# linusmossberg/monte-carlo-ray-tracer

Hardware: NVIDIA H100
Metric: Mray/s (primary+shadow+bounce) (higher is better)
Workload: dtype f64

## Files before the change

include/mcrt_abi.h:

```cpp
#ifndef MCRT_ABI_H
#define MCRT_ABI_H

#include <stddef.h>
#include <stdint.h>

#ifdef __cplusplus
extern "C" {
#endif

#define MCRT_ABI_VERSION 1

typedef enum mcrt_status {
    MCRT_OK = 0,
    MCRT_ERR_INVALID = -1,
    MCRT_ERR_CUDA = -2,
    MCRT_ERR_NO_SCENE = -3,
    MCRT_ERR_UNSUPPORTED = -4,
    MCRT_ERR_NO_PHOTONS = -5
} mcrt_status;

enum { MCRT_PRIM_TRIANGLE = 0, MCRT_PRIM_SPHERE = 1, MCRT_PRIM_QUADRIC = 2 };

enum { MCRT_INTEGRATOR_PATH = 0, MCRT_INTEGRATOR_PHOTON = 1 };

// ... 47 lines not shown
    const uint32_t* light_prim;
    const double* light_cdf;
    double scene_ior;
} mcrt_scene_desc;

typedef struct mcrt_camera {
    double eye[3], forward[3], left[3], up[3];
    double focal_length, sensor_width, aperture_radius, focus_distance;
    uint32_t width, height;
    uint32_t thin_lens;
    uint32_t _pad;
} mcrt_camera;

typedef struct mcrt_ray {
    double origin[3];
    double direction[3];
} mcrt_ray;

typedef struct mcrt_hit {
    double t, u, v;
    uint32_t prim;
    uint32_t interpolate;
} mcrt_hit;

typedef struct mcrt_photon_map_desc {
    uint32_t n_octants;
    const double* octant_bounds;
    const uint64_t* octant_start;
    const uint64_t* octant_count;
    const uint32_t* octant_next_sibling;
    const uint8_t* octant_leaf;
    uint64_t n_photons;
    const float* photons;
} mcrt_photon_map_desc;

typedef struct mcrt_stats {
    uint64_t paths;
    uint64_t extension_rays;
    uint64_t shadow_rays;
    uint64_t box_tests;
    uint64_t prim_tests;
    uint64_t knn_queries;
    uint64_t wavefront_iterations;
    uint64_t kernel_launches;
    uint64_t ior_stack_overflows;
    uint32_t max_depth;
    uint32_t _pad;
    double gpu_ms_total;
    double gpu_ms_generate, gpu_ms_extend, gpu_ms_shade, gpu_ms_shadow, gpu_ms_knn;
    uint64_t extend_launches, shadow_launches;
    uint64_t shadow_box_tests, shadow_prim_tests;
    uint64_t extend_work_sum, extend_work_warpmax;
    uint64_t replayed_rays;
} mcrt_stats;

typedef struct mcrt_ctx mcrt_ctx;

int mcrt_abi_version(void);

int mcrt_init(int device, mcrt_ctx** out_ctx);
void mcrt_destroy(mcrt_ctx* ctx);
const char* mcrt_last_error(const mcrt_ctx* ctx);

int mcrt_scene_upload(mcrt_ctx* ctx, const mcrt_scene_desc* scene, uint64_t* h2d_bytes);

int mcrt_photon_upload(mcrt_ctx* ctx, const mcrt_photon_map_desc* caustic_map,
                       const mcrt_photon_map_desc* global_map, uint32_t k_nearest,
                       uint32_t direct_visualization, uint64_t* h2d_bytes);

enum { MCRT_FILM_BOX = 0, MCRT_FILM_MITCHELL_NETRAVALI = 1, MCRT_FILM_CATMULL_ROM = 2, MCRT_FILM_B_SPLINE = 3,
       MCRT_FILM_HERMITE = 4, MCRT_FILM_GAUSSIAN = 5, MCRT_FILM_LANCZOS = 6 };
typedef struct mcrt_film {
    uint32_t filter;
    uint32_t cache_size;
    double radius;
} mcrt_film;

int mcrt_set_film(mcrt_ctx* ctx, const mcrt_film* film);

typedef struct mcrt_photon_emit_params {
    uint64_t emissions;
    double caustic_factor;
    uint32_t max_photons_per_octree_leaf;
    uint32_t k_nearest_photons;
    uint32_t direct_visualization;
    uint32_t global_seed;
    double scene_bounds[6];
} mcrt_photon_emit_params;

int mcrt_photon_emit(mcrt_ctx* ctx, const mcrt_photon_emit_params* params, int precision,
                     uint64_t* n_caustic, uint64_t* n_global, mcrt_stats* stats);

int mcrt_photon_emit_total(mcrt_ctx* ctx, const mcrt_photon_emit_params* params, uint64_t* total_emissions);
int mcrt_photon_emit_range(mcrt_ctx* ctx, const mcrt_photon_emit_params* params, int precision,
                           uint64_t work_first, uint64_t work_count, const float** caustic_dev, uint64_t* n_caustic,
                           const float** global_dev, uint64_t* n_global, mcrt_stats* stats);
int mcrt_photon_build_dev(mcrt_ctx* ctx, const mcrt_photon_emit_params* params, const float* caustic_dev,
                          uint64_t n_caustic, const float* global_dev, uint64_t n_global, double* build_ms);

int mcrt_photon_download(mcrt_ctx* ctx, int which, mcrt_photon_map_desc* out);

int mcrt_octree_build(mcrt_ctx* ctx, const float* photons, uint64_t n, uint32_t max_photons_per_octree_leaf,
                      const double* scene_bounds6, void** handle, mcrt_photon_map_desc* out, double* gpu_ms);
void mcrt_octree_free(void* handle);

typedef struct mcrt_obj_mesh {
// ... 131 lines not shown
```

monte-carlo-ray-tracer_b200/__init__.py:

```python
import ctypes as C
import math
import os
import struct

import numpy as np

HERE = os.path.dirname(os.path.abspath(__file__))
LIB_PATH = os.environ.get("MCRT_LIB", os.path.join(HERE, "libmcrt_b200.so"))

INTEGRATOR_PATH, INTEGRATOR_PHOTON = 0, 1
PRECISION_F64, PRECISION_F32 = 0, 1
PRIM_TRIANGLE, PRIM_SPHERE, PRIM_QUADRIC = 0, 1, 2
NO_PRIM = 0xFFFFFFFF

ABI_SYMBOLS = [
    "mcrt_abi_version", "mcrt_init", "mcrt_destroy", "mcrt_last_error", "mcrt_scene_upload",
    "mcrt_photon_upload", "mcrt_photon_emit", "mcrt_photon_download", "mcrt_octree_build",
    "mcrt_octree_free", "mcrt_render_rows", "mcrt_render_rows_dev", "mcrt_render_rows_strided_dev",
    "mcrt_trace_closest",
    "mcrt_sample_rays", "mcrt_sampler_stream", "mcrt_knn_search", "mcrt_set_option", "mcrt_set_film",
    "mcrt_obj_load", "mcrt_obj_free", "mcrt_obj_vertex_normals",
    "mcrt_bvh_build", "mcrt_bvh_free", "mcrt_image_tonemap", "mcrt_image_tonemap_dev",
    "mcrt_render_rows_strided_peers", "mcrt_frame_alloc", "mcrt_frame_open", "mcrt_frame_close", "mcrt_frame_free",
    "mcrt_render_film_sums_strided_dev", "mcrt_film_resolve_dev",
# ... 79 lines not shown


HIT_DTYPE = np.dtype([("t", "<f8"), ("u", "<f8"), ("v", "<f8"), ("prim", "<u4"), ("interpolate", "<u4")])


class PhotonMapDesc(C.Structure):
    _fields_ = [("n_octants", C.c_uint32), ("octant_bounds", C.c_void_p), ("octant_start", C.c_void_p),
                ("octant_count", C.c_void_p), ("octant_next_sibling", C.c_void_p), ("octant_leaf", C.c_void_p),
                ("n_photons", C.c_uint64), ("photons", C.c_void_p)]


class ImageParams(C.Structure):
    _fields_ = [("plain", C.c_uint32), ("tonemapper", C.c_uint32), ("exposure_scale", C.c_double),
                ("gain_scale", C.c_double)]

    @classmethod
    def from_json(cls, image):
        tm = str(image.get("tonemapper", "HABLE")).upper()
        return cls(int(bool(image.get("plain", False))), 1 if tm == "ACES" else 0,
                   math.pow(2, image.get("exposure_compensation", 0.0)), math.pow(2, image.get("gain_compensation", 0.0)))


class ObjMeshRec(C.Structure):
    _fields_ = [("n_vertices", C.c_uint64), ("n_normals", C.c_uint64), ("n_tri_v", C.c_uint64), ("n_tri_vt", C.c_uint64),
                ("n_tri_vn", C.c_uint64), ("vertices", C.c_void_p), ("normals", C.c_void_p), ("tri_v", C.c_void_p),
                ("tri_vt", C.c_void_p), ("tri_vn", C.c_void_p)]


class BvhDesc(C.Structure):
    _fields_ = [("n_nodes", C.c_uint32), ("n_prims", C.c_uint32), ("node_bounds", C.c_void_p),
                ("node_first_prim", C.c_void_p), ("node_prim_count", C.c_void_p), ("node_next_sibling", C.c_void_p),
                ("prim_order", C.c_void_p), ("build_rounds", C.c_uint32), ("kernel_launches", C.c_uint32)]


BVH_TYPES = {"octree": 0, "binary_sah": 1, "quaternary_sah": 2}


class PhotonEmitParams(C.Structure):
    _fields_ = [("emissions", C.c_uint64), ("caustic_factor", C.c_double), ("max_photons_per_octree_leaf", C.c_uint32),
                ("k_nearest_photons", C.c_uint32), ("direct_visualization", C.c_uint32), ("global_seed", C.c_uint32),
                ("scene_bounds", C.c_double * 6)]


class Stats(C.Structure):
    _fields_ = [("paths", C.c_uint64), ("extension_rays", C.c_uint64), ("shadow_rays", C.c_uint64),
                ("box_tests", C.c_uint64), ("prim_tests", C.c_uint64), ("knn_queries", C.c_uint64),
                ("wavefront_iterations", C.c_uint64), ("kernel_launches", C.c_uint64),
                ("ior_stack_overflows", C.c_uint64), ("max_depth", C.c_uint32), ("_pad", C.c_uint32),
                ("gpu_ms_total", C.c_double), ("gpu_ms_generate", C.c_double), ("gpu_ms_extend", C.c_double),
                ("gpu_ms_shade", C.c_double), ("gpu_ms_shadow", C.c_double), ("gpu_ms_knn", C.c_double),
                ("extend_launches", C.c_uint64), ("shadow_launches", C.c_uint64),
                ("shadow_box_tests", C.c_uint64), ("shadow_prim_tests", C.c_uint64),
                ("extend_work_sum", C.c_uint64), ("extend_work_warpmax", C.c_uint64),
                ("replayed_rays", C.c_uint64)]

    def as_dict(self):
        return {f: getattr(self, f) for f, _ in self._fields_ if not f.startswith("_")}


_lib = None


def lib():
    global _lib
    if _lib is None:
        if not os.path.exists(LIB_PATH):
            raise McrtError(f"{LIB_PATH} is missing: run `python -c 'import __graft_entry__ as g; g.build()'`")
        L = C.CDLL(LIB_PATH)
        L.mcrt_abi_version.restype = C.c_int
        L.mcrt_init.argtypes = [C.c_int, C.POINTER(C.c_void_p)]
        L.mcrt_destroy.argtypes = [C.c_void_p]
        L.mcrt_destroy.restype = None
        L.mcrt_last_error.argtypes = [C.c_void_p]
        L.mcrt_last_error.restype = C.c_char_p
        L.mcrt_scene_upload.argtypes = [C.c_void_p, C.POINTER(SceneDesc), C.POINTER(C.c_uint64)]
        L.mcrt_photon_upload.argtypes = [C.c_void_p, C.POINTER(PhotonMapDesc), C.POINTER(PhotonMapDesc),
                                         C.c_uint32, C.c_uint32, C.POINTER(C.c_uint64)]
        L.mcrt_photon_emit.argtypes = [C.c_void_p, C.POINTER(PhotonEmitParams), C.c_int, C.POINTER(C.c_uint64),
                                       C.POINTER(C.c_uint64), C.POINTER(Stats)]
        L.mcrt_photon_download.argtypes = [C.c_void_p, C.c_int, C.POINTER(PhotonMapDesc)]
        L.mcrt_octree_build.argtypes = [C.c_void_p, C.c_void_p, C.c_uint64, C.c_uint32, C.c_void_p, C.POINTER(C.c_void_p),
                                        C.POINTER(PhotonMapDesc), C.POINTER(C.c_double)]
        L.mcrt_octree_free.argtypes = [C.c_void_p]
        L.mcrt_octree_free.restype = None
        render_args = [C.c_void_p, C.POINTER(CameraRec), C.c_uint32, C.c_uint32, C.c_uint32, C.c_uint32,
                       C.c_int, C.c_int, C.c_void_p, C.POINTER(Stats)]
        L.mcrt_render_rows.argtypes = render_args
        L.mcrt_render_rows_dev.argtypes = render_args
        L.mcrt_render_rows_strided_dev.argtypes = [C.c_void_p, C.POINTER(CameraRec), C.c_uint32, C.c_uint32, C.c_uint32,
                                                   C.c_uint32, C.c_uint32, C.c_int, C.c_int, C.c_void_p, C.POINTER(Stats)]
        L.mcrt_render_rows_strided_peers.argtypes = [C.c_void_p, C.POINTER(CameraRec), C.c_uint32, C.c_uint32, C.c_uint32, C.c_uint32,
                                                     C.c_uint32, C.c_int, C.c_int, C.c_void_p, C.c_uint32, C.c_int, C.POINTER(Stats)]
        L.mcrt_frame_alloc.argtypes = [C.c_void_p, C.c_uint64, C.POINTER(C.c_void_p), C.c_void_p]
        L.mcrt_frame_open.argtypes = [C.c_void_p, C.c_void_p, C.POINTER(C.c_void_p)]
        L.mcrt_frame_close.argtypes = [C.c_void_p, C.c_void_p]
        L.mcrt_frame_free.argtypes = [C.c_void_p, C.c_void_p]
        L.mcrt_fp64_peak.argtypes = [C.c_void_p, C.POINTER(C.c_double)]
        L.mcrt_bvh4_host.argtypes = [C.POINTER(SceneDesc), C.c_uint32, C.POINTER(C.c_void_p), C.POINTER(C.c_void_p), C.POINTER(C.c_uint32)]
        L.mcrt_bvh4_host_free.argtypes = [C.c_void_p]
        L.mcrt_bvh4_host_free.restype = None
        L.mcrt_render_film_sums_strided_dev.argtypes = [C.c_void_p, C.POINTER(CameraRec), C.c_uint32, C.c_uint32, C.c_uint32, C.c_uint32,
                                                        C.c_uint32, C.c_int, C.c_int, C.c_void_p, C.c_void_p, C.POINTER(Stats)]
        L.mcrt_film_resolve_dev.argtypes = [C.c_void_p, C.c_void_p, C.c_void_p, C.c_uint64, C.c_void_p]
        L.mcrt_render_accumulate_dev.argtypes = [C.c_void_p, C.POINTER(CameraRec), C.c_uint32, C.c_uint32, C.c_uint32, C.c_uint32,
                                                 C.c_uint32, C.c_uint32, C.c_int, C.c_int, C.c_void_p, C.c_void_p, C.POINTER(Stats)]
        L.mcrt_progressive_resolve_dev.argtypes = [C.c_void_p, C.c_void_p, C.c_void_p, C.c_uint64, C.c_void_p, C.c_void_p, C.c_uint64,
                                                   C.c_uint32, C.c_uint32, C.c_uint32, C.c_void_p, C.c_void_p, C.POINTER(C.c_double)]
# ... 943 lines not shown
```

monte-carlo-ray-tracer_b200/build.py:

```python
import concurrent.futures as cf
import os
import subprocess
import sys

HERE = os.path.dirname(os.path.abspath(__file__))
CSRC = os.path.join(HERE, "csrc")
ROOT = os.path.dirname(HERE)
LIB = os.path.join(HERE, "libmcrt_b200.so")

ARCH = ["-gencode", "arch=compute_90a,code=sm_90a"]
COMMON = ["-O3", "-std=c++17", "-lineinfo", "-Xcompiler", "-fPIC", "-I", os.path.join(ROOT, "include"), "-I", CSRC]

UNITS = [
    ("kernels_f64.cu", ["--fmad=false"]),
    ("kernels_f32.cu", []),
    ("bvh_build.cu", ["--fmad=false"]),
    ("image.cu", ["--fmad=false"]),
    ("obj_abi.cu", ["--fmad=false"]),
    ("denoise.cu", ["--fmad=false"]),
    ("abi.cu", []),
]


def _run(cmd):
    r = subprocess.run(cmd, capture_output=True, text=True)
    if r.returncode != 0:
        sys.stderr.write(" ".join(cmd) + "\n" + r.stdout + r.stderr + "\n")
        raise RuntimeError("nvcc failed")
    return r.stdout + r.stderr


def build(force=False, verbose=False, defines=(), suffix=""):
    global LIB
    lib = os.path.join(HERE, f"libmcrt_b200{suffix}.so")
    objdir = os.path.join(HERE, "build" + suffix)
    os.makedirs(objdir, exist_ok=True)
    deps = [os.path.join(CSRC, f) for f in os.listdir(CSRC)] + [os.path.join(ROOT, "include", "mcrt_abi.h"),
                                                              os.path.join(HERE, "host", "obj_loader.cpp"),
                                                              os.path.join(HERE, "host", "obj_loader.hpp")]
    newest = max(os.path.getmtime(d) for d in deps)
    jobs, objs = [], []
    for src, extra in UNITS:
        obj = os.path.join(objdir, src[:-3] + ".o")
        objs.append(obj)
        if force or not os.path.exists(obj) or os.path.getmtime(obj) < newest:
            cmd = ["nvcc"] + ARCH + COMMON + list(defines) + extra + (["-Xptxas", "-v"] if verbose else []) + ["-c", os.path.join(CSRC, src), "-o", obj]
            jobs.append(cmd)
    with cf.ThreadPoolExecutor(max_workers=4) as ex:
        outs = list(ex.map(_run, jobs))
    if verbose:
        for o in outs:
            sys.stderr.write(o)
    if jobs or not os.path.exists(lib):
        _run(["nvcc"] + ARCH + ["-shared", "-o", lib] + objs + ["-Xcompiler", "-pthread"])
    return lib


if __name__ == "__main__":
    defs = [a for a in sys.argv[1:] if a.startswith("-D")]
    suf = [a.split("=", 1)[1] for a in sys.argv[1:] if a.startswith("--suffix=")]
    print(build(force="--force" in sys.argv, verbose="-v" in sys.argv, defines=defs, suffix=suf[0] if suf else ""))
```

monte-carlo-ray-tracer_b200/csrc/abi.cu:

```cuda
#include <algorithm>
#include <cmath>
#include <cstdio>
#include <cstdlib>
#include <cstring>
#include <string>
#include <vector>

#include "mcrt_abi.h"
#include "launch.h"
#include "bvh_build.h"
#include "image.h"
#include "denoise.h"

using namespace mcrt;

static const int MCRT_INTERNAL_EMIT = 100;

#define CK(call)                                                                              \
    do {                                                                                      \
        cudaError_t e_ = (call);                                                              \
        if (e_ != cudaSuccess)                                                                \
        {                                                                                     \
            ctx->error = std::string(#call) + ": " + cudaGetErrorString(e_);                  \
            return MCRT_ERR_CUDA;                                                             \
// ... 534 lines not shown
        if ((rc = devAlloc(ctx, ctx->sort_allocs, &r.shade_rank, n))) return rc;
        if ((rc = devAlloc(ctx, ctx->sort_allocs, &r.shade_order, n))) return rc;
        if ((rc = devAlloc(ctx, ctx->sort_allocs, &r.hist_shade, (size_t)SORT_BINS))) return rc;
        if ((rc = devAlloc(ctx, ctx->sort_allocs, &r.hist_path, (size_t)SORT_BINS))) return rc;
        if ((rc = devAlloc(ctx, ctx->sort_allocs, &r.hist_shadow, (size_t)SORT_BINS))) return rc;
        if ((rc = devAlloc(ctx, ctx->sort_allocs, &r.bin_start, (size_t)SORT_BINS))) return rc;
        if ((rc = devAlloc(ctx, ctx->sort_allocs, &r.block_offset, (size_t)2 * SORT_SCAN_BLOCKS))) return rc;
        if ((rc = devAlloc(ctx, ctx->sort_allocs, &r.done_counter, (size_t)1))) return rc;
        CK(cudaMemset(r.done_counter, 0, sizeof(uint32_t)));
        ctx->sort_capacity = ctx->pool_paths;
        return MCRT_OK;
    }

    int ensureFilm(mcrt_ctx* ctx, size_t values)
    {
        if (ctx->film_values >= values && ctx->d_film) return MCRT_OK;
        if (ctx->d_film) cudaFree(ctx->d_film);
        ctx->d_film = nullptr; ctx->film_values = 0;
        CK(cudaMalloc((void**)&ctx->d_film, values * sizeof(double)));
        ctx->film_values = values;
        return MCRT_OK;
    }

    template <class R> DeviceScene<R>& sceneOf(mcrt_ctx* ctx);
    template <> DeviceScene<double>& sceneOf<double>(mcrt_ctx* ctx) { return ctx->scene64; }
    template <> DeviceScene<float>& sceneOf<float>(mcrt_ctx* ctx) { return ctx->scene32; }
    template <class R> WaveBuffers<R>& waveOf(mcrt_ctx* ctx);
    template <> WaveBuffers<double>& waveOf<double>(mcrt_ctx* ctx) { return ctx->wave64; }
    template <> WaveBuffers<float>& waveOf<float>(mcrt_ctx* ctx) { return ctx->wave32; }
    template <class R> std::vector<void*>& waveAllocsOf(mcrt_ctx* ctx);
    template <> std::vector<void*>& waveAllocsOf<double>(mcrt_ctx* ctx) { return ctx->wave_allocs64; }
    template <> std::vector<void*>& waveAllocsOf<float>(mcrt_ctx* ctx) { return ctx->wave_allocs32; }

    void fillStats(mcrt_stats* st, const Counters& c, uint64_t iterations, uint64_t launches, double ms)
    {
        if (!st) return;
        std::memset(st, 0, sizeof(*st));
        st->paths = c.paths;
        st->extension_rays = c.extension_rays;
        st->shadow_rays = c.shadow_rays;
        st->box_tests = c.box_tests;
        st->prim_tests = c.prim_tests;
        st->knn_queries = c.knn_queries;
        st->wavefront_iterations = iterations;
        st->kernel_launches = launches;
        st->ior_stack_overflows = c.ior_stack_overflows;
        st->max_depth = c.max_depth;
        st->gpu_ms_total = ms;
        st->shadow_box_tests = c.shadow_box_tests;
        st->shadow_prim_tests = c.shadow_prim_tests;
        st->extend_work_sum = c.work_sum;
        st->extend_work_warpmax = c.work_warpmax;
        st->replayed_rays = c.replayed_rays;
    }

    template <class R> DeviceCamera<R> deviceCamera(const mcrt_camera& cam)
    {
        DeviceCamera<R> c;
        std::memset(&c, 0, sizeof(c));
        c.eye = v3<R>(cam.eye); c.forward = v3<R>(cam.forward);
        c.left = v3<R>(cam.left); c.up = v3<R>(cam.up);
        c.focal_length = (R)cam.focal_length; c.sensor_width = (R)cam.sensor_width;
        c.aperture_radius = (R)cam.aperture_radius; c.focus_distance = (R)cam.focus_distance;
        c.width = cam.width; c.height = cam.height; c.thin_lens = cam.thin_lens;
        return c;
    }

    struct FilmSums
    {
        double* rgb;
        double* wsum;
    };

    template <class R>
    int runWavefront(mcrt_ctx* ctx, const mcrt_camera* cam, uint32_t row_first, uint32_t row_step, uint32_t n_pixels, uint32_t spp,
                     uint64_t total_work, uint32_t global_seed, int integrator, const double* d_user_rays,
                     const uint32_t* d_user_pixel, const uint32_t* d_user_sample, size_t film_pixels,
                     double film_weight, double* out_dev, mcrt_stats* stats, uint32_t sample_first = 0,
                     const FilmSums* accum = nullptr, const uint32_t* d_pixel_list = nullptr)
    {
        if (!ctx->has_scene) { ctx->error = "no scene uploaded"; return MCRT_ERR_NO_SCENE; }
        if (integrator == MCRT_INTEGRATOR_PHOTON && !ctx->has_photons)
        {
            ctx->error = "photon-mapped render requested without mcrt_photon_upload";
            return MCRT_ERR_NO_PHOTONS;
        }
        WaveBuffers<R>& wb = waveOf<R>(ctx);
        int rc;
        if ((rc = ensureWave(ctx, wb, waveAllocsOf<R>(ctx)))) return rc;
        if (!accum && (rc = ensureFilm(ctx, film_pixels * 3))) return rc;
        const bool filtered = cam && !d_user_rays && !ctx->film_default && integrator != MCRT_INTERNAL_EMIT;
        if (filtered && !accum && ctx->film_wsum_values < film_pixels)
        {
            if (ctx->d_film_wsum) cudaFree(ctx->d_film_wsum);
            ctx->d_film_wsum = nullptr; ctx->film_wsum_values = 0;
            CK(cudaMalloc((void**)&ctx->d_film_wsum, film_pixels * sizeof(double)));
            ctx->film_wsum_values = film_pixels;
        }
        KnnQuery<R>* knn_queue = nullptr;
        const uint32_t knn_capacity = 2u * ctx->pool_paths;
        if (integrator == MCRT_INTEGRATOR_PHOTON)
        {
            void*& q = Mode<R>::parity ? ctx->knn_queue64 : ctx->knn_queue32;
            uint32_t& cap = Mode<R>::parity ? ctx->knn_capacity64 : ctx->knn_capacity32;
            if (cap != knn_capacity)
            {
// ... 1464 lines not shown
```

monte-carlo-ray-tracer_b200/csrc/bvh4.cuh:

```cuda
#pragma once

#include "intersect.cuh"

#ifndef MCRT_FAST_STACK
#define MCRT_FAST_STACK 40
#endif
#ifndef MCRT_SPECULATIVE
#define MCRT_SPECULATIVE 0
#endif
#ifndef MCRT_FAST_SMEM_STACK
#define MCRT_FAST_SMEM_STACK 0
#endif

namespace mcrt
{
    constexpr uint32_t BVH4_LEAF = 0x80000000u;
    constexpr uint32_t BVH4_MAX_PRIMS = 1u << 23;
    constexpr int FAST_STACK = MCRT_FAST_STACK;
    constexpr int FAST_SMEM_STACK = MCRT_FAST_SMEM_STACK;
    constexpr int FAST_LOCAL_STACK = FAST_STACK - FAST_SMEM_STACK;
    inline size_t fastStackSharedBytes(int block_threads) { return (size_t)FAST_SMEM_STACK * block_threads * sizeof(uint2); }

    struct alignas(16) Bvh4Node
    {
// ... 223 lines not shown
                    if (!have_cur) break;
                }
                else
                {
                    have_cur = visitNode(sc, cnt, overflow);
                    if (!have_cur) break;
                }
                if (stashed && !__any_sync(__activemask(), stashed == 0u)) break;
            }
            if (stashed && !testLeaf(stashed, sc, ray, cnt)) return false;
            return have_cur;
#else
            while (!(cur & BVH4_LEAF))
            {
                if (!visitNode(sc, cnt, overflow)) return false;
            }
            if (!testLeaf(cur, sc, ray, cnt)) return false;
            return pop();
#endif
        }

        MCRT_D bool ambiguous(const DeviceScene<double>& sc) const
        {
            if (degenerate) return true;
            return best.prim != NO_PRIM && (best.interpolate != 0u || second_t <= best.t + ambiguityDelta(best.t, (double)sc.scene_scale));
        }
    };

    template <int PRIMS>
    MCRT_D Hit<double> traverseFast(const DeviceScene<double>& sc, const RayQ<double>& ray, TraceCounters& cnt,
                                    uint32_t& overflow, bool& ambiguous)
    {
        FastSearch<PRIMS> fs;
        fs.begin(ray);
        while (fs.step(sc, ray, cnt, overflow)) { }
        ambiguous = fs.ambiguous(sc);
        return fs.best;
    }

    template <int PRIMS>
    __device__ __noinline__ void traceReferenceOrderOutOfLine(const DeviceScene<double>* sc, const RayQ<double>* ray, Hit<double>* out,
                                                              uint32_t* box_tests, uint32_t* prim_tests, uint32_t* overflow)
    {
        TraceCounters c = { 0u, 0u };
        uint32_t ov = 0;
        *out = traverseReferenceOrder<PRIMS>(*sc, *ray, c, ov);
        *box_tests += c.box_tests; *prim_tests += c.prim_tests;
        if (ov) *overflow = 1;
    }

#ifndef MCRT_FETCH_THRESHOLD
#define MCRT_FETCH_THRESHOLD 22
#endif
    template <int PRIMS, bool OCC = false, class Load, class Done>
    MCRT_D void traceManyFast(const DeviceScene<double>& sc, uint32_t n, uint32_t* fetch_counter, Load load, Done done,
                              TraceCounters& cnt, uint32_t& overflow)
    {
        FastSearch<PRIMS, OCC> fs;
        RayQ<double> ray;
        uint32_t item = 0;
        bool active = false;
        bool more = true;
        const unsigned lane = threadIdx.x & 31u;
        while (true)
        {
            const unsigned need = __ballot_sync(0xFFFFFFFFu, !active);
            if (need && more)
            {
                uint32_t base = 0;
                const int leader = __ffs(need) - 1;
                if ((int)lane == leader) base = atomicAdd(fetch_counter, (uint32_t)__popc(need));
                base = __shfl_sync(0xFFFFFFFFu, base, leader);
                more = base < n;
                if (!active)
                {
                    const uint32_t ii = base + (uint32_t)__popc(need & ((1u << lane) - 1u));
                    if (ii < n)
                    {
                        if constexpr (OCC)
                        {
                            uint32_t target;
                            item = load(ii, ray, target);
                            if (fs.beginOcclusion(sc, ray, target, cnt)) { active = true; if (fs.verdict == 2u) fs.sp = 0, fs.cur = BVH4_LEAF; }
                            else { Hit<double> miss = fs.best; miss.prim = NO_PRIM; done(item, ray, miss); }
                        }
                        else
                        {
                            item = load(ii, ray);
                            fs.begin(ray);
                            active = true;
                        }
                    }
                }
            }
            if (__ballot_sync(0xFFFFFFFFu, active) == 0u)
            {
                if (!more) break;
                continue;
            }
            while (active)
            {
                if (!fs.step(sc, ray, cnt, overflow))
                {
                    Hit<double> h = fs.best;
                    bool replay;
                    if constexpr (OCC) { replay = fs.verdict == 2u; if (fs.verdict == 1u) h.prim = NO_PRIM; }
                    else replay = fs.ambiguous(sc);
                    if (replay)
                    {
                        const DeviceScene<double> sc_copy = sc;
                        RayQ<double> rq_copy = ray;
                        rq_copy.inv_d = 1.0 / ray.d;
                        Hit<double> h2;
                        traceReferenceOrderOutOfLine<PRIMS>(&sc_copy, &rq_copy, &h2, &cnt.box_tests, &cnt.prim_tests, &overflow);
                        h = h2;
                        cnt.replayed++;
                    }
                    done(item, ray, h);
                    active = false;
                    break;
                }
                if (__popc(__activemask()) < MCRT_FETCH_THRESHOLD) break;
            }
        }
    }
}
```

monte-carlo-ray-tracer_b200/csrc/integrator.cuh:

```cuda
#pragma once

#include "bsdf.cuh"
#include "intersect.cuh"
#include "bvh4.cuh"
#include "photon.cuh"
#include "film.cuh"

#ifndef MCRT_TRACE_MINBLOCKS_F64
#define MCRT_TRACE_MINBLOCKS_F64 2
#endif
#ifndef MCRT_TRACE_MINBLOCKS_F32
#define MCRT_TRACE_MINBLOCKS_F32 4
#endif
#ifndef MCRT_TRACE_MINBLOCKS_F64_PRUNED
#define MCRT_TRACE_MINBLOCKS_F64_PRUNED 4
#endif
#ifndef MCRT_TRACE_MINBLOCKS_FAST
#define MCRT_TRACE_MINBLOCKS_FAST 2
#endif
#ifndef MCRT_TRACE_MINBLOCKS_DYN
#define MCRT_TRACE_MINBLOCKS_DYN 4
#endif
#ifndef MCRT_KNN_MINBLOCKS
#define MCRT_KNN_MINBLOCKS 8
#endif
#ifndef MCRT_SHADE_MINBLOCKS
#define MCRT_SHADE_MINBLOCKS 3
#endif
#ifndef MCRT_SHADE_MINBLOCKS_LITE
#define MCRT_SHADE_MINBLOCKS_LITE 3
#endif
#ifndef MCRT_SORT_ORIGIN_BITS
#define MCRT_SORT_ORIGIN_BITS 4
#endif
#ifndef MCRT_SORT_DIR_Q
#define MCRT_SORT_DIR_Q 1
#endif

namespace mcrt
{
    constexpr int IOR_STACK_CAPACITY = 8;

    struct Counters
    {
        uint32_t n_cur, n_next, n_shadow, n_gen;
        unsigned long long next_work, total_work;
        unsigned long long paths, extension_rays, shadow_rays, box_tests, prim_tests, knn_queries;
        unsigned long long shadow_box_tests, shadow_prim_tests;
        unsigned long long ior_stack_overflows;
        unsigned long long replayed_rays;
        uint32_t fetch_extend, fetch_shadow;
        uint32_t traversal_overflow, max_depth;
        uint32_t n_knn, _pad;
        unsigned long long work_sum, work_warpmax;
        unsigned long long n_photons[2];
        uint32_t photon_overflow, _pad2;
    };

    template <class R> struct PathBuffer
    {
        V4<R>* ray_o;
        V4<R>* ray_d;
        V4<R>* thr;
        V4<R>* iors_a;
        V4<R>* iors_b;
        uint4* meta;
        uint4* meta2;
    };

    template <class R> struct alignas(16 * sizeof(R)) ShadowRecord
    {
        V4<R> o;
        V4<R> d;
        uint4 meta;
        V4<R> k;
    };
    static_assert(sizeof(ShadowRecord<double>) == 128 && sizeof(ShadowRecord<float>) == 64, "one shadow record per line");
    static_assert(offsetof(ShadowRecord<double>, k) == 96, "the float64 padding is the 16-byte chunk 5 (k_shade writes it)");

    constexpr uint32_t SORT_ORIGIN_BITS = MCRT_SORT_ORIGIN_BITS;
    constexpr uint32_t SORT_DIR_Q = MCRT_SORT_DIR_Q;
    constexpr uint32_t SORT_DIR_BITS = 3 + 2 * SORT_DIR_Q;
    constexpr uint32_t SORT_KEY_BITS = 3 * SORT_ORIGIN_BITS + SORT_DIR_BITS;
    constexpr uint32_t SORT_BINS = 1u << SORT_KEY_BITS;

    struct RaySort
    {
        uint32_t* path_key[2];
        uint32_t* path_rank[2];
        uint32_t* path_order;
        uint32_t* shadow_key;
        uint32_t* shadow_rank;
        uint32_t* shadow_order;
        uint32_t* hist_path;
        uint32_t* hist_shadow;
        uint32_t* bin_start;
        uint32_t* block_offset;
        uint32_t* done_counter;
        uint32_t shade_sorted;
        uint32_t* shade_key;
        uint32_t* shade_rank;
        uint32_t* shade_order;
        uint32_t* hist_shade;
        uint32_t prim_scale;
        float key_min[3], key_scale[3];
    };

    MCRT_D uint32_t spreadBits3(uint32_t v)
    {
// ... 276 lines not shown
            const unsigned long long w = base_work + j;
            uint32_t pixel, sample, film_index;
            V3<R> start, direction;
            if (p.user_rays)
            {
                pixel = p.user_pixel[w];
                sample = p.user_sample[w];
                film_index = (uint32_t)w;
                const double* r = p.user_rays + 6 * w;
                start = V3<R>((R)r[0], (R)r[1], (R)r[2]);
                direction = V3<R>((R)r[3], (R)r[4], (R)r[5]);
            }
            else
            {
                uint32_t local = (uint32_t)(w % p.n_pixels);
                if constexpr (LIST) local = p.pixel_list[local];
                sample = (uint32_t)(w / p.n_pixels);
                const uint32_t row = local / p.camera.width, col = local - row * p.camera.width;
                pixel = (p.row_first + row * p.row_step) * p.camera.width + col;
                film_index = local;
                SamplerState smp = SamplerState::make(p.global_seed, pixel, sample, 0u);
                cameraRay(p.camera, p.scene.scene_ior, pixel, smp, start, direction);
                if constexpr (FILM) filmSplatSampleWeight(p.filmp, p.global_seed, pixel, sample);
            }
            stStream(&out.ray_o[slot], V4<R>(start, p.scene.scene_ior));
            stStream(&out.ray_d[slot], V4<R>(direction, R(1)));
            stStream(&out.thr[slot], V4<R>(R(1), R(1), R(1), R(0)));
            stStream(&out.meta[slot], make_uint4(pixel, sample, 0u, 0u));
            stStream(&out.meta2[slot], make_uint4(NO_PRIM, 1u, film_index, NO_PRIM));
            if (p.sort.path_order) key = rayKey(p.sort, start, direction, NO_PRIM);
            }
            if (p.sort.path_order)
            {
                const uint32_t rank = sortRank(p.sort.hist_path, key, valid);
                if (valid) { p.sort.path_key[next][slot] = key; p.sort.path_rank[next][slot] = rank; }
            }
        }
    }

    static __global__ void k_advance(Counters* c)
    {
        c->n_cur = c->n_next + c->n_gen;
        c->next_work += c->n_gen;
        c->paths += c->n_gen;
        c->n_next = 0;
        c->n_gen = 0;
        c->n_shadow = 0;
        c->n_knn = 0;
        c->fetch_extend = 0;
        c->fetch_shadow = 0;
    }

    template <class R, int PRIMS, int FAST>
    __global__ void __launch_bounds__(256, FAST == 2 ? MCRT_TRACE_MINBLOCKS_DYN : (FAST == 1 ? MCRT_TRACE_MINBLOCKS_FAST : (PRIMS == PRIMS_ALL ? Mode<R>::trace_minblocks : Mode<R>::trace_minblocks_pruned))) k_extend(WaveParams<R> p, int cur)
    {
        const uint32_t n = p.counters->n_cur;
        const PathBuffer<R>& in = p.buf[cur];
        TraceCounters cnt = { 0u, 0u, 0u };
        uint32_t overflow = 0;
        unsigned long long rays = 0;
        const uint32_t* order = p.sort.path_order;
        if constexpr (Mode<R>::parity && FAST == 2)
        {
            traceManyFast<PRIMS>(p.scene, n, &p.counters->fetch_extend,
                [&](uint32_t ii, RayQ<R>& r)
                {
                    const uint32_t i = order ? order[ii] : ii;
                    const V4<R> ro = ldStream(&in.ray_o[i]), rd = ldStream(&in.ray_d[i]);
                    r.o = ro.xyz(); r.d = rd.xyz();
                    if constexpr (PRIMS == PRIMS_ALL) r.inv_d = R(1) / r.d;
                    return i;
                },
                [&](uint32_t i, const RayQ<R>&, const Hit<R>& h)
                {
                    stStream(&p.hits[i], V4<R>(h.t, h.u, h.v, h.prim == NO_PRIM ? R(-1) : R(h.prim)));
                    rays++;
                }, cnt, overflow);
            flushStats(p.counters, cnt, rays, false, overflow);
            return;
        }
        for (uint32_t ii = blockIdx.x * blockDim.x + threadIdx.x; ii < n; ii += gridDim.x * blockDim.x)
        {
            const uint32_t i = order ? order[ii] : ii;
            const V4<R> ro = ldStream(&in.ray_o[i]);
            const V4<R> rd = ldStream(&in.ray_d[i]);
            uint32_t skip = NO_PRIM;
            if constexpr (!Mode<R>::parity) skip = in.meta2[i].w;
#ifdef MCRT_TAIL_DIAGNOSTIC
            const uint32_t w0 = cnt.box_tests + cnt.prim_tests;
#endif
            Hit<R> h = traceClosest<PRIMS, FAST != 0>(p.scene, ro.xyz(), rd.xyz(), skip, cnt, overflow);
            stStream(&p.hits[i], V4<R>(h.t, h.u, h.v, h.prim == NO_PRIM ? R(-1) : R(h.prim)));
            rays++;
#ifdef MCRT_TAIL_DIAGNOSTIC
            const uint32_t w = cnt.box_tests + cnt.prim_tests - w0;
            const unsigned am = __activemask();
            const uint32_t wmax = __reduce_max_sync(am, w);
            atomicAdd(&p.counters->work_sum, (unsigned long long)w);
            if ((threadIdx.x & 31u) == (unsigned)(__ffs(am) - 1)) atomicAdd(&p.counters->work_warpmax, 32ull * wmax);
#endif
        }
        flushStats(p.counters, cnt, rays, false, overflow);
    }

    template <class R>
    MCRT_D void sampleLightPoint(const Light<R>& l, R u, R v, V3<R>& pos, V3<R>& normal)
    {
        if (l.type == PRIM_TRIANGLE)
        {
            R su = msqrt(u);
            pos = (R(1) - su) * l.p0 + (R(1) - v) * su * l.p1 + v * su * l.p2;
            normal = l.normal;
        }
        else
        {
            R z = R(1) - R(2) * u;
            R r = msqrt(R(1) - pow2(z));
            R phi = Consts<R>::TWO_PI * v;
            R sn, cs;
            msincos(phi, &sn, &cs);
            pos = l.p0 + l.p1.x * V3<R>(r * cs, r * sn, z);
            normal = (pos - l.p0) / l.p1.x;
        }
    }

    template <class R> MCRT_D R powerHeuristic(R a_pdf, R b_pdf)
    {
        R a2 = a_pdf * a_pdf;
        return a2 / (a2 + b_pdf * b_pdf);
    }
// ... 255 lines not shown
                pkey = rayKey(p.sort, nray.start, nray.direction, hit_prim);
                prank = atomicAdd(&p.sort.hist_path[pkey], 1u);
            }
            if (sorting && want_shadow)
            {
                skey = rayKey(p.sort, sh_o, sh_d, hit_prim);
                srank = atomicAdd(&p.sort.hist_shadow[skey], 1u);
            }
            if (alive)
            {
                stStream(&out.ray_o[slot], V4<R>(nray.start, nray.medium_ior));
                stStream(&out.ray_d[slot], V4<R>(nray.direction, nray.refraction_scale));
                stStream(&out.thr[slot], V4<R>(throughput, ls_bsdf_pdf));
                if (ior_count > 1)
                {
                    out.iors_a[slot] = V4<R>(iors[1], iors[2], iors[3], iors[4]);
                    if (ior_count > 5) out.iors_b[slot] = V4<R>(iors[5], iors[6], iors[7], R(0));
                }
                stStream(&out.meta[slot], make_uint4(meta.x, meta.y, (nray.depth & 0xFFFFu) | (nray.diffuse_depth << 16),
                                                     (uint32_t)nray.refraction_level));
                stStream(&out.meta2[slot], make_uint4(ls_light, ior_count | (nray.dirac_delta ? 256u : 0u), meta2.z,
                                                      sc.shade[hit_prim].type == PRIM_TRIANGLE ? hit_prim : NO_PRIM));
                if (sorting) { p.sort.path_key[cur ^ 1][slot] = pkey; p.sort.path_rank[cur ^ 1][slot] = prank; }
            }
            if (want_shadow)
            {
                ShadowRecord<R>& srec = p.shadow[sslot];
                stStream(&srec.o, V4<R>(sh_o, sh_bsdf_pdf));
                stStream(&srec.d, V4<R>(sh_d, sh_area_cos));
                stStream(&srec.meta, make_uint4(sh_light, meta2.z, sc.shade[hit_prim].type == PRIM_TRIANGLE ? hit_prim : NO_PRIM, meta.y));
                if constexpr (sizeof(R) == 8) stStream(reinterpret_cast<uint4*>(&srec) + 5, make_uint4(0u, 0u, 0u, 0u));
                stStream(&srec.k, V4<R>(sh_k, sh_select));
                if (sorting) { p.sort.shadow_key[sslot] = skey; p.sort.shadow_rank[sslot] = srank; }
            }

            if constexpr (KIND == 1)
            {
                const uint32_t q0 = warpAppend(&c->n_knn, want_knn >= 1);
                if (want_knn >= 1 && q0 < p.pm.query_capacity) p.pm.queries[q0] = knn_q;
                const uint32_t q1 = warpAppend(&c->n_knn, want_knn == 2);
                if (want_knn == 2 && q1 < p.pm.query_capacity)
                {
                    knn_q.meta.z |= 2u;
                    p.pm.queries[q1] = knn_q;
                }
            }
        }

        if (local_max_depth) atomicMax(&c->max_depth, local_max_depth);
        if (stack_overflows) atomicAdd(&c->ior_stack_overflows, (unsigned long long)stack_overflows);
    }

    template <class R, bool FILM, int PRIMS, int FAST>
    __global__ void __launch_bounds__(256, FAST == 2 ? MCRT_TRACE_MINBLOCKS_DYN : (FAST == 1 ? MCRT_TRACE_MINBLOCKS_FAST : (PRIMS == PRIMS_ALL ? Mode<R>::trace_minblocks : Mode<R>::trace_minblocks_pruned))) k_shadow(WaveParams<R> p)
    {
        const uint32_t n = p.counters->n_shadow;
        TraceCounters cnt = { 0u, 0u, 0u };
        uint32_t overflow = 0;
        unsigned long long rays = 0;
        const uint32_t* order = p.sort.shadow_order;
        if constexpr (Mode<R>::parity && FAST == 2)
        {
            traceManyFast<PRIMS, true>(p.scene, n, &p.counters->fetch_shadow,
                [&](uint32_t ii, RayQ<R>& r, uint32_t& target)
                {
                    const uint32_t i = order ? order[ii] : ii;
                    const V4<R> so = ldStream(&p.shadow[i].o), sd = ldStream(&p.shadow[i].d);
                    r.o = so.xyz(); r.d = sd.xyz();
                    if constexpr (PRIMS == PRIMS_ALL) r.inv_d = R(1) / r.d;
                    target = p.shadow[i].meta.x;
                    return i;
                },
                [&](uint32_t i, const RayQ<R>&, const Hit<R>& h)
                {
                    rays++;
                    const ShadowRecord<R>& srec = p.shadow[i];
                    const uint4 sm = srec.meta;
                    if (h.prim == sm.x)
                    {
                        const V4<R> so = srec.o, sd = srec.d, sk = srec.k;
                        R light_pdf = pow2(h.t) / sd.w;
                        R mis_weight = powerHeuristic(light_pdf, so.w);
                        depositRadiance<FILM>(p, sm.y, pixelOfFilmIndex(p, sm.y), sm.w, sk.xyz() * (mis_weight / (light_pdf * sk.w)));
                    }
                }, cnt, overflow);
            flushStats(p.counters, cnt, rays, true, overflow);
            return;
        }
        for (uint32_t ii = blockIdx.x * blockDim.x + threadIdx.x; ii < n; ii += gridDim.x * blockDim.x)
        {
            const uint32_t i = order ? order[ii] : ii;
            const ShadowRecord<R>& srec = p.shadow[i];
            const V4<R> so = ldStream(&srec.o), sd = ldStream(&srec.d);
            const uint4 sm = ldStream(&srec.meta);
            Hit<R> h;
            if constexpr (Mode<R>::parity && FAST != 0) h = traceVisible<PRIMS>(p.scene, so.xyz(), sd.xyz(), sm.x, cnt, overflow);
            else h = traceClosest<PRIMS, false>(p.scene, so.xyz(), sd.xyz(), sm.z, cnt, overflow);
            rays++;
            if (h.prim == sm.x)
            {
                const V4<R> sk = srec.k;
                R light_pdf = pow2(h.t) / sd.w;
                R mis_weight = powerHeuristic(light_pdf, so.w);
                depositRadiance<FILM>(p, sm.y, pixelOfFilmIndex(p, sm.y), sm.w, sk.xyz() * (mis_weight / (light_pdf * sk.w)));
            }
        }
        flushStats(p.counters, cnt, rays, true, overflow);
    }



    constexpr uint32_t SHADE_CLASS_BINS = 64;

    template <class R>
    __global__ void __launch_bounds__(256) k_shade_key(WaveParams<R> p)
    {
        __shared__ uint32_t s_hist[SHADE_CLASS_BINS], s_base[SHADE_CLASS_BINS];
        const uint32_t n = p.counters->n_cur;
        const uint32_t chunks = (n + 255u) / 256u;
        for (uint32_t chunk = blockIdx.x; chunk < chunks; chunk += gridDim.x)
        {
            if (threadIdx.x < SHADE_CLASS_BINS) s_hist[threadIdx.x] = 0u;
            __syncthreads();
            const uint32_t i = chunk * 256u + threadIdx.x;
            uint32_t key = 0, local = 0;
            if (i < n)
            {
                const R w = p.hits[i].w;
                if (!(w < R(0))) key = p.scene.shade_class[(uint32_t)w];
                local = atomicAdd(&s_hist[key], 1u);
            }
            __syncthreads();
            if (threadIdx.x < SHADE_CLASS_BINS && s_hist[threadIdx.x]) s_base[threadIdx.x] = atomicAdd(&p.sort.hist_shade[threadIdx.x], s_hist[threadIdx.x]);
            __syncthreads();
            if (i < n) { p.sort.shade_key[i] = key; p.sort.shade_rank[i] = s_base[key] + local; }
            __syncthreads();
        }
    }

    constexpr uint32_t SORT_SCAN_BLOCKS = SORT_BINS / 1024;

    static __global__ void __launch_bounds__(256) k_sort_scan(uint32_t* hist, uint32_t* bin_start, uint32_t* block_offset,
                                                              uint32_t* done_counter)
    {
        __shared__ uint32_t warp_sums[8];
        __shared__ uint32_t is_last;
        const uint32_t t = threadIdx.x, base = blockIdx.x * 1024u + t * 4u;
        const uint4 v = *reinterpret_cast<const uint4*>(hist + base);
        *reinterpret_cast<uint4*>(hist + base) = make_uint4(0u, 0u, 0u, 0u);
        const uint32_t sum = v.x + v.y + v.z + v.w;
        uint32_t incl = sum;
// ... 496 lines not shown
```

monte-carlo-ray-tracer_b200/csrc/kernels_impl.cuh:

```cuda
#include "launch.h"

namespace mcrt
{
    template <> void Launch<MCRT_REAL>::generate(const WaveParams<MCRT_REAL>& p, int next, int grid, cudaStream_t s)
    {
        if (p.pixel_list)
        {
            if (p.filmp.is_default_box) k_generate<MCRT_REAL, false, true><<<grid, 256, 0, s>>>(p, next);
            else k_generate<MCRT_REAL, true, true><<<grid, 256, 0, s>>>(p, next);
            return;
        }
        if (p.filmp.is_default_box) k_generate<MCRT_REAL, false, false><<<grid, 256, 0, s>>>(p, next);
        else k_generate<MCRT_REAL, true, false><<<grid, 256, 0, s>>>(p, next);
    }
    template <> void Launch<MCRT_REAL>::extend(const WaveParams<MCRT_REAL>& p, int cur, int grid, cudaStream_t s)
    {
        if constexpr (Mode<MCRT_REAL>::parity)
        {
            if (p.scene.bvh4 && p.scene.dynamic_fetch)
            {
                if (p.scene.prims_class == PRIMS_TRI) k_extend<MCRT_REAL, PRIMS_TRI, 2><<<grid, 256, fastStackSharedBytes(256), s>>>(p, cur);
                else if (p.scene.prims_class == PRIMS_TRI_SPHERE) k_extend<MCRT_REAL, PRIMS_TRI_SPHERE, 2><<<grid, 256, fastStackSharedBytes(256), s>>>(p, cur);
                else k_extend<MCRT_REAL, PRIMS_ALL, 2><<<grid, 256, fastStackSharedBytes(256), s>>>(p, cur);
                return;
            }
            if (p.scene.bvh4)
            {
                if (p.scene.prims_class == PRIMS_TRI) k_extend<MCRT_REAL, PRIMS_TRI, 1><<<grid, 256, fastStackSharedBytes(256), s>>>(p, cur);
                else if (p.scene.prims_class == PRIMS_TRI_SPHERE) k_extend<MCRT_REAL, PRIMS_TRI_SPHERE, 1><<<grid, 256, fastStackSharedBytes(256), s>>>(p, cur);
                else k_extend<MCRT_REAL, PRIMS_ALL, 1><<<grid, 256, fastStackSharedBytes(256), s>>>(p, cur);
                return;
            }
        }
        if (p.scene.prims_class == PRIMS_TRI) k_extend<MCRT_REAL, PRIMS_TRI, 0><<<grid, 256, 0, s>>>(p, cur);
        else if (p.scene.prims_class == PRIMS_TRI_SPHERE) k_extend<MCRT_REAL, PRIMS_TRI_SPHERE, 0><<<grid, 256, 0, s>>>(p, cur);
        else k_extend<MCRT_REAL, PRIMS_ALL, 0><<<grid, 256, 0, s>>>(p, cur);
    }
    template <> void Launch<MCRT_REAL>::shade(const WaveParams<MCRT_REAL>& p, int cur, int grid, cudaStream_t s)
    {
        const bool lite = (p.scene.material_flags_any & ~SHADE_FEATS_LITE) == 0;
        if (!p.filmp.is_default_box) k_shade<MCRT_REAL, 0, true, SHADE_FEATS_ALL><<<grid * 2, 128, 0, s>>>(p, cur);
        else if (lite) k_shade<MCRT_REAL, 0, false, SHADE_FEATS_LITE><<<grid * 2, 128, 0, s>>>(p, cur);
        else k_shade<MCRT_REAL, 0, false, SHADE_FEATS_ALL><<<grid * 2, 128, 0, s>>>(p, cur);
    }
    template <> void Launch<MCRT_REAL>::shadePhoton(const WaveParams<MCRT_REAL>& p, int cur, int grid, cudaStream_t s)
    {
        const bool lite = (p.scene.material_flags_any & ~SHADE_FEATS_LITE) == 0;
        if (!p.filmp.is_default_box) k_shade<MCRT_REAL, 1, true, SHADE_FEATS_ALL><<<grid * 2, 128, 0, s>>>(p, cur);
        else if (lite) k_shade<MCRT_REAL, 1, false, SHADE_FEATS_LITE><<<grid * 2, 128, 0, s>>>(p, cur);
        else k_shade<MCRT_REAL, 1, false, SHADE_FEATS_ALL><<<grid * 2, 128, 0, s>>>(p, cur);
    }
    template <> void Launch<MCRT_REAL>::knn(const WaveParams<MCRT_REAL>& p, int grid, cudaStream_t s)
    {
        const dim3 g(grid * 2), b(32 * KNN_WARPS_PER_BLOCK);
        const size_t smem = knnSharedBytes(p.pm.k_nearest);
        if (!p.filmp.is_default_box)
        {
            static bool attr_set = false;
            if (!attr_set) { cudaFuncSetAttribute(k_knn<MCRT_REAL, 0, true, SHADE_FEATS_ALL>, cudaFuncAttributeMaxDynamicSharedMemorySize, (int)knnSharedBytes(1024)); attr_set = true; }
            k_knn<MCRT_REAL, 0, true, SHADE_FEATS_ALL><<<g, b, smem, s>>>(p);
            return;
        }
        const bool lite = (p.scene.material_flags_any & ~SHADE_FEATS_LITE) == 0;
        const int slots = knnSlotsFor(p.pm.k_nearest);
        #define MCRT_KNN_LAUNCH1(SL, FE) \
            do { static bool attr_set = false; \
                 if (!attr_set) { cudaFuncSetAttribute(k_knn<MCRT_REAL, SL, false, FE>, cudaFuncAttributeMaxDynamicSharedMemorySize, (int)knnSharedBytes(1024)); attr_set = true; } \
                 k_knn<MCRT_REAL, SL, false, FE><<<g, b, smem, s>>>(p); } while (0)
        #define MCRT_KNN_LAUNCH(SL) \
            do { if (lite) MCRT_KNN_LAUNCH1(SL, SHADE_FEATS_LITE); else MCRT_KNN_LAUNCH1(SL, SHADE_FEATS_ALL); } while (0)
        switch (slots)
        {
            case 1: MCRT_KNN_LAUNCH(1); break;
            case 2: MCRT_KNN_LAUNCH(2); break;
            case 4: MCRT_KNN_LAUNCH(4); break;
            case 8: MCRT_KNN_LAUNCH(8); break;
            default: MCRT_KNN_LAUNCH(0); break;
        }
        #undef MCRT_KNN_LAUNCH
        #undef MCRT_KNN_LAUNCH1
    }
    template <> void Launch<MCRT_REAL>::shadow(const WaveParams<MCRT_REAL>& p, int grid, cudaStream_t s)
    {
// ... 56 lines not shown
```

Measured before the change: 2727.

## Fetch persistent-thread work in per-warp chunks and retune trace kernel occupancy

The persistent traversal loop now grabs fixed chunks of ray indices per warp via one atomic and keeps the leftover range in shared memory, instead of one atomic per refill sized to idle lanes. Occlusion rays that resolve immediately now go through the common step path rather than finishing inline, and the early-exit refill check is skipped once no work remains. Launch-bounds min-blocks for dynamic-fetch kernels is lowered for non-triangle scenes, the fast extend grid is scaled up, and optional tail-diagnostic counters plus build-path changes are added. This cuts atomic contention but risks coarser load balance at the tail and different register pressure.

```diff
diff --git a/include/mcrt_abi.h b/include/mcrt_abi.h
--- a/include/mcrt_abi.h
+++ b/include/mcrt_abi.h
@@ -123,6 +123,9 @@
     uint64_t shadow_box_tests, shadow_prim_tests;
     uint64_t extend_work_sum, extend_work_warpmax;
     uint64_t replayed_rays;
+    uint64_t shadow_work_sum, shadow_work_warpmax;
+    uint64_t extend_lane_steps_active, extend_lane_steps_slots;
+    uint64_t shadow_lane_steps_active, shadow_lane_steps_slots;
 } mcrt_stats;
 
 typedef struct mcrt_ctx mcrt_ctx;
diff --git a/monte-carlo-ray-tracer_b200/__init__.py b/monte-carlo-ray-tracer_b200/__init__.py
--- a/monte-carlo-ray-tracer_b200/__init__.py
+++ b/monte-carlo-ray-tracer_b200/__init__.py
@@ -155,7 +155,10 @@
                 ("extend_launches", C.c_uint64), ("shadow_launches", C.c_uint64),
                 ("shadow_box_tests", C.c_uint64), ("shadow_prim_tests", C.c_uint64),
                 ("extend_work_sum", C.c_uint64), ("extend_work_warpmax", C.c_uint64),
-                ("replayed_rays", C.c_uint64)]
+                ("replayed_rays", C.c_uint64),
+                ("shadow_work_sum", C.c_uint64), ("shadow_work_warpmax", C.c_uint64),
+                ("extend_lane_steps_active", C.c_uint64), ("extend_lane_steps_slots", C.c_uint64),
+                ("shadow_lane_steps_active", C.c_uint64), ("shadow_lane_steps_slots", C.c_uint64)]
 
     def as_dict(self):
         return {f: getattr(self, f) for f, _ in self._fields_ if not f.startswith("_")}
diff --git a/monte-carlo-ray-tracer_b200/build.py b/monte-carlo-ray-tracer_b200/build.py
--- a/monte-carlo-ray-tracer_b200/build.py
+++ b/monte-carlo-ray-tracer_b200/build.py
@@ -9,7 +9,7 @@
 LIB = os.path.join(HERE, "libmcrt_b200.so")
 
 ARCH = ["-gencode", "arch=compute_90a,code=sm_90a"]
-COMMON = ["-O3", "-std=c++17", "-lineinfo", "-Xcompiler", "-fPIC", "-I", os.path.join(ROOT, "include"), "-I", CSRC]
+COMMON = ["-O3", "-std=c++17", "-lineinfo", "-Xcompiler", "-fPIC"]
 
 UNITS = [
     ("kernels_f64.cu", ["--fmad=false"]),
@@ -30,21 +30,25 @@
     return r.stdout + r.stderr
 
 
-def build(force=False, verbose=False, defines=(), suffix=""):
+def build(force=False, verbose=False, defines=(), suffix="", src=ROOT, outdir=None):
     global LIB
-    lib = os.path.join(HERE, f"libmcrt_b200{suffix}.so")
-    objdir = os.path.join(HERE, "build" + suffix)
+    pkg = os.path.join(src, os.path.basename(HERE))
+    csrc = os.path.join(pkg, "csrc")
+    out = outdir or pkg
+    lib = os.path.join(out, f"libmcrt_b200{suffix}.so")
+    objdir = os.path.join(out, "build" + suffix)
     os.makedirs(objdir, exist_ok=True)
-    deps = [os.path.join(CSRC, f) for f in os.listdir(CSRC)] + [os.path.join(ROOT, "include", "mcrt_abi.h"),
-                                                              os.path.join(HERE, "host", "obj_loader.cpp"),
-                                                              os.path.join(HERE, "host", "obj_loader.hpp")]
+    common = COMMON + ["-I", os.path.join(src, "include"), "-I", csrc]
+    deps = [os.path.join(csrc, f) for f in os.listdir(csrc)] + [os.path.join(src, "include", "mcrt_abi.h"),
+                                                              os.path.join(pkg, "host", "obj_loader.cpp"),
+                                                              os.path.join(pkg, "host", "obj_loader.hpp")]
     newest = max(os.path.getmtime(d) for d in deps)
     jobs, objs = [], []
-    for src, extra in UNITS:
-        obj = os.path.join(objdir, src[:-3] + ".o")
+    for unit, extra in UNITS:
+        obj = os.path.join(objdir, unit[:-3] + ".o")
         objs.append(obj)
         if force or not os.path.exists(obj) or os.path.getmtime(obj) < newest:
-            cmd = ["nvcc"] + ARCH + COMMON + list(defines) + extra + (["-Xptxas", "-v"] if verbose else []) + ["-c", os.path.join(CSRC, src), "-o", obj]
+            cmd = ["nvcc"] + ARCH + common + list(defines) + extra + (["-Xptxas", "-v"] if verbose else []) + ["-c", os.path.join(csrc, unit), "-o", obj]
             jobs.append(cmd)
     with cf.ThreadPoolExecutor(max_workers=4) as ex:
         outs = list(ex.map(_run, jobs))
diff --git a/monte-carlo-ray-tracer_b200/csrc/abi.cu b/monte-carlo-ray-tracer_b200/csrc/abi.cu
--- a/monte-carlo-ray-tracer_b200/csrc/abi.cu
+++ b/monte-carlo-ray-tracer_b200/csrc/abi.cu
@@ -610,6 +610,12 @@
         st->extend_work_sum = c.work_sum;
         st->extend_work_warpmax = c.work_warpmax;
         st->replayed_rays = c.replayed_rays;
+        st->shadow_work_sum = c.shadow_work_sum;
+        st->shadow_work_warpmax = c.shadow_work_warpmax;
+        st->extend_lane_steps_active = c.extend_lane_steps[0];
+        st->extend_lane_steps_slots = c.extend_lane_steps[1];
+        st->shadow_lane_steps_active = c.shadow_lane_steps[0];
+        st->shadow_lane_steps_slots = c.shadow_lane_steps[1];
     }
 
     template <class R> DeviceCamera<R> deviceCamera(const mcrt_camera& cam)
diff --git a/monte-carlo-ray-tracer_b200/csrc/bvh4.cuh b/monte-carlo-ray-tracer_b200/csrc/bvh4.cuh
--- a/monte-carlo-ray-tracer_b200/csrc/bvh4.cuh
+++ b/monte-carlo-ray-tracer_b200/csrc/bvh4.cuh
@@ -299,37 +299,54 @@
 #ifndef MCRT_FETCH_THRESHOLD
 #define MCRT_FETCH_THRESHOLD 22
 #endif
+#ifndef MCRT_FETCH_CHUNK
+#define MCRT_FETCH_CHUNK 128
+#endif
     template <int PRIMS, bool OCC = false, class Load, class Done>
     MCRT_D void traceManyFast(const DeviceScene<double>& sc, uint32_t n, uint32_t* fetch_counter, Load load, Done done,
-                              TraceCounters& cnt, uint32_t& overflow)
+                              TraceCounters& cnt, uint32_t& overflow, unsigned long long* lane_steps)
     {
         FastSearch<PRIMS, OCC> fs;
         RayQ<double> ray;
         uint32_t item = 0;
         bool active = false;
-        bool more = true;
+        __shared__ uint2 warp_range[32];
         const unsigned lane = threadIdx.x & 31u;
+        uint2& range = warp_range[threadIdx.x >> 5];
+        if (lane == 0u) range = make_uint2(0u, 0u);
+        __syncwarp();
+#ifdef MCRT_TAIL_DIAGNOSTIC
+        unsigned long long diag_active = 0, diag_slots = 0;
+#endif
         while (true)
         {
-            const unsigned need = __ballot_sync(0xFFFFFFFFu, !active);
-            if (need && more)
-            {
-                uint32_t base = 0;
-                const int leader = __ffs(need) - 1;
-                if ((int)lane == leader) base = atomicAdd(fetch_counter, (uint32_t)__popc(need));
-                base = __shfl_sync(0xFFFFFFFFu, base, leader);
-                more = base < n;
+            uint32_t lo = range.x, hi = range.y;
+            unsigned need;
+            while ((need = __ballot_sync(0xFFFFFFFFu, !active)) != 0u && (lo < hi || hi < n))
+            {
+                if (lo == hi)
+                {
+                    uint32_t base = 0;
+                    if (lane == 0u) base = atomicAdd(fetch_counter, (uint32_t)MCRT_FETCH_CHUNK);
+                    base = __shfl_sync(0xFFFFFFFFu, base, 0);
+                    lo = min(base, n);
+                    hi = n - lo < (uint32_t)MCRT_FETCH_CHUNK ? n : lo + (uint32_t)MCRT_FETCH_CHUNK;
+                    if (lo == hi) break;
+                }
+                const uint32_t take = min((uint32_t)__popc(need), hi - lo);
                 if (!active)
                 {
-                    const uint32_t ii = base + (uint32_t)__popc(need & ((1u << lane) - 1u));
-                    if (ii < n)
+                    const uint32_t rank = (uint32_t)__popc(need & ((1u << lane) - 1u));
+                    if (rank < take)
                     {
+                        const uint32_t ii = lo + rank;
                         if constexpr (OCC)
                         {
                             uint32_t target;
                             item = load(ii, ray, target);
-                            if (fs.beginOcclusion(sc, ray, target, cnt)) { active = true; if (fs.verdict == 2u) fs.sp = 0, fs.cur = BVH4_LEAF; }
-                            else { Hit<double> miss = fs.best; miss.prim = NO_PRIM; done(item, ray, miss); }
+                            if (!fs.beginOcclusion(sc, ray, target, cnt)) fs.verdict = 1u;
+                            if (fs.verdict != 0u) fs.sp = 0, fs.cur = BVH4_LEAF;
+                            active = true;
                         }
                         else
                         {
@@ -339,14 +356,20 @@
                         }
                     }
                 }
-            }
-            if (__ballot_sync(0xFFFFFFFFu, active) == 0u)
-            {
-                if (!more) break;
-                continue;
-            }
+                lo += take;
+            }
+            if (__ballot_sync(0xFFFFFFFFu, active) == 0u) break;
+            const bool refill = lo < hi || hi < n;
+            if (lane == 0u) range = make_uint2(lo, hi);
+            __syncwarp();
             while (active)
             {
+#ifdef MCRT_TAIL_DIAGNOSTIC
+                {
+                    const unsigned am = __activemask();
+                    if (lane == (unsigned)(__ffs(am) - 1)) { diag_active += (unsigned long long)__popc(am); diag_slots += 32ull; }
+                }
+#endif
                 if (!fs.step(sc, ray, cnt, overflow))
                 {
                     Hit<double> h = fs.best;
@@ -367,8 +390,11 @@
                     active = false;
                     break;
                 }
-                if (__popc(__activemask()) < MCRT_FETCH_THRESHOLD) break;
-            }
-        }
+                if (refill && __popc(__activemask()) < MCRT_FETCH_THRESHOLD) break;
+            }
+        }
+#ifdef MCRT_TAIL_DIAGNOSTIC
+        if (diag_slots) { atomicAdd(&lane_steps[0], diag_active); atomicAdd(&lane_steps[1], diag_slots); }
+#endif
     }
 }
diff --git a/monte-carlo-ray-tracer_b200/csrc/integrator.cuh b/monte-carlo-ray-tracer_b200/csrc/integrator.cuh
--- a/monte-carlo-ray-tracer_b200/csrc/integrator.cuh
+++ b/monte-carlo-ray-tracer_b200/csrc/integrator.cuh
@@ -19,7 +19,13 @@
 #define MCRT_TRACE_MINBLOCKS_FAST 2
 #endif
 #ifndef MCRT_TRACE_MINBLOCKS_DYN
-#define MCRT_TRACE_MINBLOCKS_DYN 4
+#define MCRT_TRACE_MINBLOCKS_DYN 2
+#endif
+#ifndef MCRT_TRACE_MINBLOCKS_DYN_TRI
+#define MCRT_TRACE_MINBLOCKS_DYN_TRI 4
+#endif
+#ifndef MCRT_EXTEND_GRID_SCALE
+#define MCRT_EXTEND_GRID_SCALE 4
 #endif
 #ifndef MCRT_KNN_MINBLOCKS
 #define MCRT_KNN_MINBLOCKS 8
@@ -55,6 +61,8 @@
         unsigned long long work_sum, work_warpmax;
         unsigned long long n_photons[2];
         uint32_t photon_overflow, _pad2;
+        unsigned long long shadow_work_sum, shadow_work_warpmax;
+        unsigned long long extend_lane_steps[2], shadow_lane_steps[2];
     };
 
     template <class R> struct PathBuffer
@@ -437,7 +445,7 @@
     }
 
     template <class R, int PRIMS, int FAST>
-    __global__ void __launch_bounds__(256, FAST == 2 ? MCRT_TRACE_MINBLOCKS_DYN : (FAST == 1 ? MCRT_TRACE_MINBLOCKS_FAST : (PRIMS == PRIMS_ALL ? Mode<R>::trace_minblocks : Mode<R>::trace_minblocks_pruned))) k_extend(WaveParams<R> p, int cur)
+    __global__ void __launch_bounds__(256, FAST == 2 ? (PRIMS == PRIMS_TRI ? MCRT_TRACE_MINBLOCKS_DYN_TRI : MCRT_TRACE_MINBLOCKS_DYN) : (FAST == 1 ? MCRT_TRACE_MINBLOCKS_FAST : (PRIMS == PRIMS_ALL ? Mode<R>::trace_minblocks : Mode<R>::trace_minblocks_pruned))) k_extend(WaveParams<R> p, int cur)
     {
         const uint32_t n = p.counters->n_cur;
         const PathBuffer<R>& in = p.buf[cur];
@@ -460,7 +468,7 @@
                 {
                     stStream(&p.hits[i], V4<R>(h.t, h.u, h.v, h.prim == NO_PRIM ? R(-1) : R(h.prim)));
                     rays++;
-                }, cnt, overflow);
+                }, cnt, overflow, p.counters->extend_lane_steps);
             flushStats(p.counters, cnt, rays, false, overflow);
             return;
         }
@@ -822,7 +830,7 @@
     }
 
     template <class R, bool FILM, int PRIMS, int FAST>
-    __global__ void __launch_bounds__(256, FAST == 2 ? MCRT_TRACE_MINBLOCKS_DYN : (FAST == 1 ? MCRT_TRACE_MINBLOCKS_FAST : (PRIMS == PRIMS_ALL ? Mode<R>::trace_minblocks : Mode<R>::trace_minblocks_pruned))) k_shadow(WaveParams<R> p)
+    __global__ void __launch_bounds__(256, FAST == 2 ? (PRIMS == PRIMS_TRI ? MCRT_TRACE_MINBLOCKS_DYN_TRI : MCRT_TRACE_MINBLOCKS_DYN) : (FAST == 1 ? MCRT_TRACE_MINBLOCKS_FAST : (PRIMS == PRIMS_ALL ? Mode<R>::trace_minblocks : Mode<R>::trace_minblocks_pruned))) k_shadow(WaveParams<R> p)
     {
         const uint32_t n = p.counters->n_shadow;
         TraceCounters cnt = { 0u, 0u, 0u };
@@ -853,7 +861,7 @@
                         R mis_weight = powerHeuristic(light_pdf, so.w);
                         depositRadiance<FILM>(p, sm.y, pixelOfFilmIndex(p, sm.y), sm.w, sk.xyz() * (mis_weight / (light_pdf * sk.w)));
                     }
-                }, cnt, overflow);
+                }, cnt, overflow, p.counters->shadow_lane_steps);
             flushStats(p.counters, cnt, rays, true, overflow);
             return;
         }
@@ -863,10 +871,22 @@
             const ShadowRecord<R>& srec = p.shadow[i];
             const V4<R> so = ldStream(&srec.o), sd = ldStream(&srec.d);
             const uint4 sm = ldStream(&srec.meta);
+#ifdef MCRT_TAIL_DIAGNOSTIC
+            const uint32_t w0 = cnt.box_tests + cnt.prim_tests;
+#endif
             Hit<R> h;
             if constexpr (Mode<R>::parity && FAST != 0) h = traceVisible<PRIMS>(p.scene, so.xyz(), sd.xyz(), sm.x, cnt, overflow);
             else h = traceClosest<PRIMS, false>(p.scene, so.xyz(), sd.xyz(), sm.z, cnt, overflow);
             rays++;
+#ifdef MCRT_TAIL_DIAGNOSTIC
+            {
+                const uint32_t w = cnt.box_tests + cnt.prim_tests - w0;
+                const unsigned am = __activemask();
+                const uint32_t wmax = __reduce_max_sync(am, w);
+                atomicAdd(&p.counters->shadow_work_sum, (unsigned long long)w);
+                if ((threadIdx.x & 31u) == (unsigned)(__ffs(am) - 1)) atomicAdd(&p.counters->shadow_work_warpmax, 32ull * wmax);
+            }
+#endif
             if (h.prim == sm.x)
             {
                 const V4<R> sk = srec.k;
diff --git a/monte-carlo-ray-tracer_b200/csrc/kernels_impl.cuh b/monte-carlo-ray-tracer_b200/csrc/kernels_impl.cuh
--- a/monte-carlo-ray-tracer_b200/csrc/kernels_impl.cuh
+++ b/monte-carlo-ray-tracer_b200/csrc/kernels_impl.cuh
@@ -26,9 +26,10 @@
             }
             if (p.scene.bvh4)
             {
-                if (p.scene.prims_class == PRIMS_TRI) k_extend<MCRT_REAL, PRIMS_TRI, 1><<<grid, 256, fastStackSharedBytes(256), s>>>(p, cur);
-                else if (p.scene.prims_class == PRIMS_TRI_SPHERE) k_extend<MCRT_REAL, PRIMS_TRI_SPHERE, 1><<<grid, 256, fastStackSharedBytes(256), s>>>(p, cur);
-                else k_extend<MCRT_REAL, PRIMS_ALL, 1><<<grid, 256, fastStackSharedBytes(256), s>>>(p, cur);
+                const int g = grid * MCRT_EXTEND_GRID_SCALE;
+                if (p.scene.prims_class == PRIMS_TRI) k_extend<MCRT_REAL, PRIMS_TRI, 1><<<g, 256, fastStackSharedBytes(256), s>>>(p, cur);
+                else if (p.scene.prims_class == PRIMS_TRI_SPHERE) k_extend<MCRT_REAL, PRIMS_TRI_SPHERE, 1><<<g, 256, fastStackSharedBytes(256), s>>>(p, cur);
+                else k_extend<MCRT_REAL, PRIMS_ALL, 1><<<g, 256, fastStackSharedBytes(256), s>>>(p, cur);
                 return;
             }
         }
```

After: 2758, median of 6. 1.01x the previous value.
